# consilience-dev/llm-map-reduce-summarizer

Hardware: AMD Instinct MI355X
Metric: chunks/sec (whole node) + end-to-end wall-clock, 10h transcript, Llama-3-8B (higher is better)
Workload: dtype bf16

## Files before the change

### llm_map_reduce_summarizer_amd/csrc/kernels/stream_gemm.hip

```cpp
#include "ar_common.h"

namespace {
enum { EPI_BF16 = 0, EPI_F32_PARTIAL = 1, EPI_SWIGLU = 2, EPI_SWIGLU_SPLIT = 3, EPI_RESID_SPLIT = 4 };
constexpr int SS_PARTS = 8;
constexpr int KBLK = 128;
constexpr int LDS_XTRA = 3 * 1024;
constexpr int LDS_BUDGET = 160 * 1024 - LDS_XTRA;

struct NormArgs {
    const float* ssq;
    int ssq_tiles;
    float inv_k, eps;
    bf16* resid;
    int ldr;
    float* ssp;
    int slab_m;
    mrsum_ar::TPPush tp;
};

template <int N>
__device__ __forceinline__ void wait_vmcnt() {
    static_assert(N >= 0 && N < 64, "vmcnt range");
    __builtin_amdgcn_s_waitcnt((N & 15) | (7 << 4) | (15 << 8) | ((N >> 4) << 14));
}
// ... 560 lines not shown
        case 6: L8(MT_, EPI_, 6); break;            \
        case 7: L8(MT_, EPI_, 7); break;            \
        default: L8(MT_, EPI_, 8); break;           \
    }
#define BY_EPI8(MT_)                                                      \
    if (epi == EPI_BF16) { BY_WPB8(MT_, EPI_BF16) }                       \
    else if (epi == EPI_F32_PARTIAL) { BY_WPB8(MT_, EPI_F32_PARTIAL) }    \
    else if (epi == EPI_SWIGLU) { BY_WPB8(MT_, EPI_SWIGLU) }              \
    else if (epi == EPI_SWIGLU_SPLIT) { BY_WPB8(MT_, EPI_SWIGLU_SPLIT) }  \
    else { BY_WPB8(MT_, EPI_RESID_SPLIT) }
    switch (mt) {
        case 1: BY_EPI8(1); break;
        case 2: BY_EPI8(2); break;
        case 3: BY_EPI8(3); break;
        default: BY_EPI8(4); break;
    }
#undef BY_EPI8
#undef BY_WPB8
#undef L8
    return (int)hipGetLastError();
}

namespace {
constexpr int P14_TILE = 3584, P14_NIB = 2048, P14_TWO = 3072;
typedef unsigned int u32x2 __attribute__((ext_vector_type(2)));

template <int AUX = 0>
__device__ __forceinline__ void glds4(const void* g, char* lds) {
    __builtin_amdgcn_global_load_lds((const __attribute__((address_space(1))) void*)g,
                                     (__attribute__((address_space(3))) void*)lds, 4, 0, AUX);
}

template <int Q>
__device__ __forceinline__ uint32_t p14_hi4(uint32_t q4, uint32_t s2, uint32_t base4) {
    constexpr int SS = Q == 3 ? 7 : Q;
    const uint32_t c5 = q4 | ((s2 << Q) & 0x10101010u);
    const uint32_t nz = (c5 + 0x1f1f1f1fu) & 0x20202020u;
    const uint32_t on = (nz << 3) - (nz >> 5);
    return (c5 + (on & base4)) | ((s2 << SS) & 0x80808080u);
}

template <int PAR>
__device__ __forceinline__ bf16x8 p14_frag(uint32_t l0, uint32_t l1, uint32_t nb, uint32_t s2, uint32_t base4) {
    const uint32_t h0 = p14_hi4<2 * PAR>(nb & 0x0f0f0f0fu, s2, base4);
    const uint32_t h1 = p14_hi4<2 * PAR + 1>((nb >> 4) & 0x0f0f0f0fu, s2, base4);
    const u32x4 o = {__builtin_amdgcn_perm(h0, l0, 0x05010400u), __builtin_amdgcn_perm(h0, l0, 0x07030602u),
                     __builtin_amdgcn_perm(h1, l1, 0x05010400u), __builtin_amdgcn_perm(h1, l1, 0x07030602u)};
    return __builtin_bit_cast(bf16x8, o);
}
}

template <int MT, int EPI, int WPB>
__global__ __launch_bounds__(64 * WPB, 1) void stream_p14_kernel(const bf16* __restrict__ x, int ldx,
                                                                 const unsigned char* __restrict__ W, int base7,
                                                                 int K, int M, void* __restrict__ out, int ldo,
                                                                 int kper, float* __restrict__ parts,
                                                                 int* __restrict__ counters, const NormArgs e) {
    constexpr int R = 16 * WPB, BM = 16 * MT;
    constexpr int WBYTES = WPB * P14_TILE, SLOT = WBYTES + BM * 256;
    constexpr int D = (LDS_BUDGET / SLOT) < 8 ? (LDS_BUDGET / SLOT) : 8;
    static_assert(D >= 2, "ring too shallow");
    constexpr int XP = 2 * BM / 8;
    constexpr int XI = (XP + WPB - 1) / WPB;
    constexpr int NI = 5 + XI;
    static_assert(NI * (D - 2) < 64, "vmcnt range");
    __shared__ __attribute__((aligned(1024))) char lds[D * SLOT + LDS_XTRA];
    float* const s_ss = reinterpret_cast<float*>(lds + D * SLOT + 1024);

    const int tid = threadIdx.x, lane = tid & 63, w = tid >> 6;
    const int n0 = blockIdx.x * R;
    const int ks = blockIdx.y * kper;
    const int nkb = kper / KBLK;

    const unsigned char* const wsrc = W + ((size_t)(n0 / 16 + w) * (K / KBLK) + ks / KBLK) * P14_TILE;
    const int prow = lane >> 3, pslot = lane & 7;
    const bf16* xsrc[XI];
    int xdst[XI];
#pragma unroll
    for (int i = 0; i < XI; ++i) {
        const int q = w + WPB * i;
        const int qq = q < XP ? q : 0;
        const int row = 8 * (qq >> 1) + prow;
        xsrc[i] = x + (size_t)min(row, M - 1) * ldx + ks + 8 * (8 * (qq & 1) + (pslot ^ prow));
        xdst[i] = q < XP ? WBYTES + q * 1024 : -1;
    }
#define ISSUE14(slot, kb)                                                                            \
    {                                                                                                \
        char* base = lds + (slot) * SLOT;                                                            \
        char* wb = base + w * P14_TILE;                                                              \
        const unsigned char* ws = wsrc + (size_t)(kb) * P14_TILE;                                    \
        glds16<2>(ws + 16 * lane, wb);                                                               \
        glds16<2>(ws + 1024 + 16 * lane, wb + 1024);                                                 \
        glds16<2>(ws + P14_NIB + 16 * lane, wb + P14_NIB);                                           \
        glds4<2>(ws + P14_TWO + 4 * lane, wb + P14_TWO);                                             \
        glds4<2>(ws + P14_TWO + 256 + 4 * lane, wb + P14_TWO + 256);                                 \
        _Pragma("unroll") for (int i = 0; i < XI; ++i)                                               \
            glds16(xsrc[i] + (kb) * KBLK, xdst[i] >= 0 ? base + xdst[i] : lds + D * SLOT);           \
    }

    f32x4 acc[MT];
#pragma unroll
    for (int m = 0; m < MT; ++m) acc[m] = f32x4{0.f, 0.f, 0.f, 0.f};

#pragma unroll
    for (int s = 0; s < D - 1; ++s) ISSUE14(s, min(s, nkb - 1));

    const uint32_t base4 = (uint32_t)(base7 - 1) * 0x01010101u;
    const int r = lane & 15, g = lane >> 4;
    for (int j = 0; j < nkb; ++j) {
        if (j + D - 2 < nkb) wait_vmcnt<NI * (D - 2)>();
        else wait_vmcnt<0>();
        raw_barrier();
        if (j + D - 1 < nkb) ISSUE14((j + D - 1) % D, j + D - 1);
        const char* wl = lds + (j % D) * SLOT + w * P14_TILE;
        const char* xl = lds + (j % D) * SLOT + WBYTES;
        const u32x4 lo0 = *reinterpret_cast<const u32x4*>(wl + 16 * lane);
        const u32x4 lo1 = *reinterpret_cast<const u32x4*>(wl + 1024 + 16 * lane);
        const u32x4 nb = *reinterpret_cast<const u32x4*>(wl + P14_NIB + 16 * lane);
        const u32x2 s2 = *reinterpret_cast<const u32x2*>(wl + P14_TWO + 8 * lane);
        bf16x8 av[4];
        av[0] = p14_frag<0>(lo0[0], lo0[1], nb[0], s2.x, base4);
        av[1] = p14_frag<1>(lo0[2], lo0[3], nb[1], s2.x, base4);
        av[2] = p14_frag<0>(lo1[0], lo1[1], nb[2], s2.y, base4);
        av[3] = p14_frag<1>(lo1[2], lo1[3], nb[3], s2.y, base4);
#pragma unroll
        for (int i = 0; i < 4; ++i) {
#pragma unroll
            for (int m = 0; m < MT; ++m) {
                const u32x4 bv = *reinterpret_cast<const u32x4*>(xl + img_off(16 * m + r, 4 * i + g));
                acc[m] = __builtin_amdgcn_mfma_f32_16x16x32_bf16(av[i], __builtin_bit_cast(bf16x8, bv), acc[m], 0, 0, 0);
            }
        }
    }
#undef ISSUE14

    stream_epilogue<MT, EPI, WPB>(acc, lds, s_ss, n0, M, out, ldo, parts, counters, e);
}

MRSUM_API int mrsum_stream_p14(const void* x, int ldx, const void* W, int base7, int N, int K, int M, void* out,
                               int ldo, int epi, int splits, int wpb, void* parts, int* counters, const float* ssq,
                               int ssq_tiles, float eps, void* resid, int ldr, float* ssp, void* ar, hipStream_t s) {
    if (M <= 0) return 0;
    if (wpb < 4 || wpb > 8 || M > 64 || K % KBLK || N % (16 * wpb) || splits < 1 || (K / KBLK) % splits ||
        epi < EPI_BF16 || epi > EPI_RESID_SPLIT || base7 < 1 || base7 > 97 || ar)
        return (int)hipErrorInvalidValue;
    const bool split_epi = epi == EPI_SWIGLU_SPLIT || epi == EPI_RESID_SPLIT;
    if (epi != EPI_F32_PARTIAL && !split_epi && splits != 1) return (int)hipErrorInvalidValue;
    if (split_epi && (!parts || !counters)) return (int)hipErrorInvalidValue;
    if (epi == EPI_RESID_SPLIT && (!resid || !ssp || ldr % 4)) return (int)hipErrorInvalidValue;
    if (ssq && (ssq_tiles <= 0 || ssq_tiles % (4 * SS_PARTS))) return (int)hipErrorInvalidValue;
    NormArgs e;
    e.ssq = ssq; e.ssq_tiles = ssq_tiles; e.inv_k = 1.f / (float)K; e.eps = eps;
    e.resid = (bf16*)resid; e.ldr = ldr; e.ssp = ssp; e.slab_m = 0;
    e.tp = mrsum_ar::tp_push_of(nullptr);
    const int kper = K / splits;
    const int mt = (M + 15) / 16;
    dim3 grid(N / (16 * wpb), splits), block(64 * wpb);
    auto X = (const bf16*)x;
    auto Wp = (const unsigned char*)W;
    auto P = (float*)parts;
#define L14(MT_, EPI_, WPB_) \
    stream_p14_kernel<MT_, EPI_, WPB_><<<grid, block, 0, s>>>(X, ldx, Wp, base7, K, M, out, ldo, kper, P, counters, e)
#define BY_WPB14(MT_, EPI_)                         \
    switch (wpb) {                                  \
        case 4: L14(MT_, EPI_, 4); break;           \
        case 5: L14(MT_, EPI_, 5); break;           \
        case 6: L14(MT_, EPI_, 6); break;           \
        case 7: L14(MT_, EPI_, 7); break;           \
        default: L14(MT_, EPI_, 8); break;          \
    }
#define BY_EPI14(MT_)                                                      \
    if (epi == EPI_BF16) { BY_WPB14(MT_, EPI_BF16) }                       \
    else if (epi == EPI_F32_PARTIAL) { BY_WPB14(MT_, EPI_F32_PARTIAL) }    \
    else if (epi == EPI_SWIGLU) { BY_WPB14(MT_, EPI_SWIGLU) }              \
    else if (epi == EPI_SWIGLU_SPLIT) { BY_WPB14(MT_, EPI_SWIGLU_SPLIT) }  \
    else { BY_WPB14(MT_, EPI_RESID_SPLIT) }
    switch (mt) {
        case 1: BY_EPI14(1); break;
        case 2: BY_EPI14(2); break;
        case 3: BY_EPI14(3); break;
        default: BY_EPI14(4); break;
    }
#undef BY_EPI14
#undef BY_WPB14
#undef L14
    return (int)hipGetLastError();
}

namespace {
__global__ __launch_bounds__(256) void p14_max_kernel(const uint4* __restrict__ W, size_t n16, int* __restrict__ stats) {
    uint32_t m = 0;
    for (size_t i = (size_t)blockIdx.x * blockDim.x + threadIdx.x; i < n16; i += (size_t)gridDim.x * blockDim.x) {
        const uint4 v = W[i];
        const uint32_t d[4] = {v.x, v.y, v.z, v.w};
#pragma unroll
        for (int c = 0; c < 4; ++c) m = max(m, max((d[c] >> 8) & 0x7fu, (d[c] >> 24) & 0x7fu));
    }
#pragma unroll
    for (int o = 32; o > 0; o >>= 1) m = max(m, (uint32_t)__shfl_xor((int)m, o, 64));
    if ((threadIdx.x & 63) == 0) atomicMax(stats, (int)m);
}

__global__ __launch_bounds__(64) void p14_pack_kernel(const bf16* __restrict__ W, int K, unsigned char* __restrict__ P,
                                                      int* __restrict__ stats) {
    const int lane = threadIdx.x, r = lane & 15, g = lane >> 4;
    const int nkb = K / KBLK;
    const size_t tile = blockIdx.x;
    const int G = (int)(tile / nkb), kb = (int)(tile % nkb);
    const int base7 = max(stats[0] - 30, 1);
    const uint4* src = reinterpret_cast<const uint4*>(W + (size_t)(16 * G + r) * K + (size_t)kb * KBLK + 8 * g);
    uint32_t lo[8], nb[4], s2[2] = {0u, 0u};
// ... 15 lines not shown
            s2[i >> 1] |= (c5 >> 4) << (8 * b + 4 - q) | sg << (8 * b + 7 - (q == 3 ? 7 : q));
        }
    }
    unsigned char* t = P + tile * P14_TILE;
    *reinterpret_cast<uint4*>(t + 16 * lane) = make_uint4(lo[0], lo[1], lo[2], lo[3]);
    *reinterpret_cast<uint4*>(t + 1024 + 16 * lane) = make_uint4(lo[4], lo[5], lo[6], lo[7]);
    *reinterpret_cast<uint4*>(t + P14_NIB + 16 * lane) = make_uint4(nb[0], nb[1], nb[2], nb[3]);
    *reinterpret_cast<uint2*>(t + P14_TWO + 8 * lane) = make_uint2(s2[0], s2[1]);
    if (bad) atomicAdd(stats + 1, bad);
}
}

MRSUM_API int mrsum_p14_pack(const void* W, int N, int K, void* packed, int* stats, hipStream_t s) {
    if (N <= 0 || K <= 0 || N % 16 || K % KBLK || !W || !packed || !stats) return (int)hipErrorInvalidValue;
    hipError_t rc = hipMemsetAsync(stats, 0, 2 * sizeof(int), s);
    if (rc != hipSuccess) return (int)rc;
    const size_t n16 = (size_t)N * K / 8;
    const int blocks = (int)((n16 + 255) / 256 < 4096 ? (n16 + 255) / 256 : 4096);
    p14_max_kernel<<<blocks, 256, 0, s>>>((const uint4*)W, n16, stats);
    p14_pack_kernel<<<(unsigned)((size_t)(N / 16) * (K / KBLK)), 64, 0, s>>>((const bf16*)W, K, (unsigned char*)packed,
                                                                              stats);
    return (int)hipGetLastError();
}
```

### llm_map_reduce_summarizer_amd/engine/model.py

```python

from __future__ import annotations

import hashlib
import math
import os
from dataclasses import dataclass
from typing import Callable, List, Optional

import torch

from .. import ops
from ..ops.reference import Fp8Weight, interleave_gate_up, rope_cos_sin
from ..parallel.dist import AsyncWorks
from .config import ModelConfig


def _seed_for(seed: int, name: str) -> int:
    return int.from_bytes(hashlib.sha1(("%d:%s" % (seed, name)).encode()).digest()[:8], "little") & ((1 << 63) - 1)


def _randn(shape, std: float, seed: int, name: str, device, dtype) -> torch.Tensor:
    g = torch.Generator(device=device)
    g.manual_seed(_seed_for(seed, name))
    t = torch.randn(*shape, generator=g, device=device, dtype=torch.float32 if device.type == "cpu" else dtype)
    t.mul_(std)
    return t.to(dtype)


# ... 142 lines not shown
            self.layers.append(LayerWeights(ones(), wqkv, wo, ones(), wgu, wd))
        self.final_norm = ones()
        lm = _randn((c.vocab_size, c.hidden), std, seed, "lm_head", dev, dt)
        v = self.vocab_local
        self.lm_head = lm[r * v:(r + 1) * v].contiguous()
        del lm
        self._quantize_lm_head()

    def _quantize_lm_head(self) -> None:
        if self.weight_dtype == "fp8" and not isinstance(self.lm_head, Fp8Weight):
            self.lm_head = Fp8Weight.quantize(self.lm_head)

    def _pack_p14(self) -> None:
        self.p14 = []
        if self.weight_dtype != "bf16" or self.tp_size != 1 or self.device.type != "cuda" \
                or self.dtype != torch.bfloat16:
            return
        hip = _hip()
        if not hip.p14_enabled():
            return
        todo = [(self.lm_head, "lm_head")]
        for lw in self.layers:
            todo += [(lw.wqkv, "qkv"), (lw.wo, "o"), (lw.wgu, "gate_up"), (lw.wdown, "down")]
        for w, role in todo:
            if hip.p14_role_used(role) and w.shape[0] % 16 == 0 and w.shape[1] % 128 == 0:
                self.p14.append(hip.p14_attach(w, role))

    def __del__(self):
        try:
            for pw in getattr(self, "p14", ()):
                _hip().p14_detach(pw.w)
        except Exception:
            pass

    def weight_bytes(self) -> int:
        def nb(t):
            return t.nbytes() if isinstance(t, Fp8Weight) else t.numel() * t.element_size()
        n = nb(self.embed) + nb(self.lm_head) + nb(self.final_norm) + sum(pw.nbytes() for pw in self.p14)
        for lw in self.layers:
            n += sum(nb(t) for t in (lw.ln1, lw.wqkv, lw.wo, lw.ln2, lw.wgu, lw.wdown))
        return n

    def local_push(self):
        if self._local_push is None:
            from ..parallel.custom_ar import LocalPush
            self._local_push = LocalPush()
        return self._local_push

    def _all_reduce(self, t: torch.Tensor) -> torch.Tensor:
        if self.tp_size > 1:
            if self.custom_ar is not None and self.custom_ar.fits(t):
                self.custom_ar.all_reduce(t)
            else:
                if t.is_cuda and torch.cuda.is_current_stream_capturing():
# ... 228 lines not shown
```

### llm_map_reduce_summarizer_amd/ops/hip.py

```python

from __future__ import annotations

import ctypes
import os
from typing import Optional

import torch

from ._lib import kernels_lib
from .reference import Fp8Weight

_c_int, _c_float, _vp = ctypes.c_int, ctypes.c_float, ctypes.c_void_p

_SIGS = {
    "mrsum_rmsnorm": [_vp, _vp, _vp, _c_int, _c_int, _c_int, _c_int, _c_float, _vp],
    "mrsum_add_rmsnorm": [_vp, _vp, _vp, _vp, _c_int, _c_int, _c_int, _c_int, _c_float, _vp],
    "mrsum_rmsnorm_fp8": [_vp, _vp, _vp, _vp, _vp, _c_int, _c_int, _c_int, _c_int, _c_float, _c_int, _vp],
    "mrsum_rope_kv": [_vp, _c_int, _c_int, _vp, _vp, _vp, _c_int, _vp, _vp, _vp, _c_int, _c_int, _c_int, _c_int,
                      _c_int, _c_int, _vp],
    "mrsum_rope_kv_parts": [_vp, _c_int, _vp, _c_int, _c_int, _vp, _vp, _vp, _c_int, _vp, _vp, _vp, _c_int,
                            _c_int, _c_int, _c_int, _c_int, _vp],
    "mrsum_swiglu": [_vp, _vp, _c_int, _c_int, _vp],
    "mrsum_kv_scatter": [_vp, _c_int, _c_int, _c_int, _vp, _vp, _vp, _vp, _c_int, _vp],
    "mrsum_embed": [_vp, _vp, _vp, _c_int, _c_int, _c_int, _vp],
    "mrsum_attn_prefill": [_vp, _c_int, _vp, _vp, _c_int, _c_int, _vp, _c_int, _c_int, _c_int, _c_int, _c_float, _vp],
    "mrsum_attn_prefill_paged": [_vp, _c_int, _vp, _vp, _c_int, _c_int, _vp, _c_int, _c_int, _c_int, _c_int, _c_float,
                                 _vp,
                                 _vp, _vp, _c_int, _vp, _vp, _c_int, _vp],
    "mrsum_attn_decode_mfma": [_vp, _c_int, _vp, _vp, _vp, _c_int, _vp, _vp, _vp, _vp, _c_int, _c_int, _c_int,
                               _c_int, _c_int, _c_int, _c_int, _c_float, _vp, _c_int, _vp],
    "mrsum_attn_decode_rope": [_vp, _c_int, _vp, _vp, _vp, _vp, _c_int, _vp, _vp, _vp, _vp, _c_int, _c_int,
                               _c_int, _c_int, _c_int, _c_int, _c_int, _c_float, _vp, _c_int, _vp],
    "mrsum_skinny_gemm": [_vp, _c_int, _vp, _c_int, _c_int, _c_int, _vp, _c_int, _c_int, _c_int, _c_int, _vp, _c_int,
                          _c_float, _vp, _c_int, _vp, _vp, _c_int, _vp],
    "mrsum_skinny_resid_capacity_w": [_c_int],
    "mrsum_skinny_lds": [_vp, _c_int, _vp, _c_int, _c_int, _c_int, _vp, _c_int, _c_int, _c_int, _c_int, _vp],
    "mrsum_stream_gemm": [_vp, _c_int, _vp, _c_int, _c_int, _c_int, _vp, _c_int, _c_int, _c_int, _c_int, _vp, _vp,
                          _vp, _c_int, _c_float, _vp, _c_int, _vp, _c_int, _vp, _vp],
    "mrsum_stream_fp8": [_vp, _c_int, _vp, _vp, _c_int, _c_int, _c_int, _vp, _c_int, _c_int, _c_int, _c_int, _vp, _vp,
                         _vp, _c_int, _c_float, _vp, _c_int, _vp, _vp, _vp],
    "mrsum_stream_p14": [_vp, _c_int, _vp, _c_int, _c_int, _c_int, _c_int, _vp, _c_int, _c_int, _c_int, _c_int, _vp,
                         _vp, _vp, _c_int, _c_float, _vp, _c_int, _vp, _vp, _vp],
    "mrsum_p14_pack": [_vp, _c_int, _c_int, _vp, _vp, _vp],
    "mrsum_skinny_fp8": [_vp, _c_int, _vp, _vp, _c_int, _c_int, _c_int, _vp, _c_int, _c_int, _c_int, _c_int, _vp,
                         _c_int, _c_float, _vp, _c_int, _vp, _vp, _c_int, _vp],
    "mrsum_skinny_fp8_resid_capacity": [],
    "mrsum_quant_fp8_rows": [_vp, _c_int, _vp, _vp, _c_int, _c_int, _vp],
    "mrsum_add_rmsnorm_parts": [_vp, _c_int, _vp, _vp, _vp, _c_int, _c_int, _c_int, _c_float, _vp],
    "mrsum_sample_keys": [_vp, _c_int, _c_int, _c_int, _c_int, _vp, _vp, _vp, _vp, _vp],
    "mrsum_sample_finish": [_vp, _vp, _vp, _vp, _vp, _vp, _c_int, _vp, _vp, _c_int, _vp],
    "mrsum_gemm": [_vp, _c_int, _vp, _c_int, _vp, _c_int, _c_int, _c_int, _c_int, _c_int, _c_int, _vp, _vp, _c_int,
                   _c_int, _vp],
    "mrsum_sample": [_vp, _c_int, _c_int, _c_int, _vp, _vp, _vp, _vp, _vp, _vp, _vp, _vp, _vp, _c_int, _vp, _vp,
                     _vp],
    "mrsum_penalize": [_vp, _c_int, _c_int, _c_int, _c_int, _vp, _c_int, _vp, _vp, _vp, _vp, _vp, _vp],
    "mrsum_penalize_scan": [_vp, _c_int, _c_int, _c_int, _c_int, _vp, _c_int, _vp, _vp, _vp, _vp, _vp, _vp],
    "mrsum_constrain": [_vp, _c_int, _c_int, _c_int, _c_int, _vp, _vp, _c_int, _vp, _vp, _vp, _vp, _vp, _vp, _vp],
    "mrsum_sample_finish_stops": [_vp, _vp, _vp, _vp, _vp, _vp, _c_int, _vp, _vp, _vp, _c_int, _vp],
    "mrsum_sample_keys_filtered": [_vp, _c_int, _c_int, _c_int, _vp, _vp, _vp, _vp, _vp, _vp, _vp, _vp, _vp, _vp],
    "mrsum_logprobs": [_vp, _c_int, _c_int, _c_int, _vp, _vp, _vp, _c_int, _vp, _vp, _vp, _vp, _vp, _vp, _vp, _vp],
    "mrsum_logprobs_pick": [_vp, _c_int, _c_int, _c_int, _vp, _c_int, _vp, _vp, _vp, _vp, _c_int, _vp],
    "mrsum_sample_thresh": [_vp, _c_int, _c_int, _c_int, _vp, _vp, _vp, _vp, _vp, _vp, _vp],
    "mrsum_sample_filtered": [_vp, _c_int, _c_int, _c_int, _vp, _vp, _vp, _vp, _vp, _vp, _vp, _vp, _vp, _vp, _vp,
                              _vp, _vp, _c_int, _vp, _vp, _vp],
}

# ... 825 lines not shown
            continue
        grid = N // (16 * wpb) * splits
        k = (round(grid / (-(-grid // N_CU) * N_CU), 3), wpb)
        if key is None or k > key:
            best, key = wpb, k
    return best


def _stream_launch(x, w, out, epi, splits, ldo, wpb, parts, counters, norm, resid, ssp, slab_m, ar=None):
    M, K = x.shape
    N = w.shape[0]
    _req(w.is_contiguous() and w.shape[1] == K, "stream_gemm: weight must be [N, K] contiguous")
    tall_ok = M <= 128 and epi in (EPI_BF16, EPI_F32_PARTIAL, EPI_SWIGLU) and norm is None
    _req(1 <= M and (M <= SKINNY_MAX_M or tall_ok) and K % 128 == 0 and 4 <= wpb <= 8 and N % (16 * wpb) == 0
         and (K // 128) % splits == 0, "stream_gemm: unsupported shape M=%d N=%d K=%d S=%d wpb=%d"
         % (M, N, K, splits, wpb))
    if epi in (EPI_SWIGLU_SPLIT, EPI_RESID_SPLIT):
        _req(parts is not None and parts.shape == (splits, M, N) and parts.dtype == torch.float32
             and counters is not None and counters.numel() >= N // (16 * wpb), "stream_gemm: split-K scratch")
    if epi == EPI_RESID_SPLIT:
        _req(ssp.shape[1] == N // (16 * wpb), "stream_gemm: ssp tiles")
    sq, tiles, eps = _norm_args(x, norm)
    rp, ldr, sp = _resid_args(x, N, epi, resid, ssp)
    pw = p14_lookup(w) if _P14 else None
    if pw is not None and M <= SKINNY_MAX_M and not slab_m and ar is None and p14_takes(pw.role, M):
        STATS["stream_p14"] += 1
        _check(_fn("mrsum_stream_p14")(_p(x), x.stride(0), _p(pw.packed), pw.base7, N, K, M, _p(out), ldo, epi, splits,
                                       wpb, _p(parts), _p(counters), sq, tiles, eps, rp, ldr, sp, None, _stream()),
               "stream_p14")
        return out
    STATS["stream_bf16"] += 1
    _check(_fn("mrsum_stream_gemm")(_p(x), x.stride(0), _p(w), N, K, M, _p(out), ldo, epi, splits, wpb, _p(parts),
                                    _p(counters), sq, tiles, eps, rp, ldr, sp, slab_m, ar, _stream()), "stream_gemm")
    return out


P14_ROLES = ("qkv", "o", "gate_up", "down", "lm_head")
_P14_PLAN = {("gate_up", 1), ("gate_up", 16), ("gate_up", 64), ("lm_head", 1), ("lm_head", 16),
             ("down", 1), ("down", 16)}
_P14 = {}


class PackedWeight:

    def __init__(self, w: torch.Tensor, packed: Optional[torch.Tensor], base7: int, packable: bool, role: str):
        self.w, self.packed, self.base7, self.packable, self.role = w, packed, base7, packable, role

    def nbytes(self) -> int:
# ... 28 lines not shown
    stats = torch.zeros(2, dtype=torch.int32, device=w.device)
    _check(_fn("mrsum_p14_pack")(_p(w), N, K, _p(packed), _p(stats), _stream()), "p14_pack")
    mx, bad = (int(v) for v in stats.tolist())
    return packed, max(mx - 30, 1), bad


def p14_attach(w: torch.Tensor, role: str) -> PackedWeight:
    _req(role in P14_ROLES, "p14_attach: unknown role %r" % (role,))
    packed, base7, bad = p14_pack(w)
    if bad:
        print("p14: %s weight %s has %d elements outside the exponent window: bf16 kernel kept"
              % (role, tuple(w.shape), bad))
        return PackedWeight(w, None, base7, False, role)
    pw = _P14[(w.data_ptr(), w.shape[0], w.shape[1])] = PackedWeight(w, packed, base7, True, role)
    return pw


def p14_detach(w: torch.Tensor) -> None:
    _P14.pop((w.data_ptr(), w.shape[0], w.shape[1]), None)


def p14_lookup(w: torch.Tensor) -> Optional[PackedWeight]:
    return _P14.get((w.data_ptr(), w.shape[0], w.shape[1]))


def linear_takes_norm(M: int, N: int, K: int) -> bool:
    return 1 <= M <= SKINNY_MAX_M and K % 128 == 0 and stream_config(N, K, splits=1) is not None


def linear(x: torch.Tensor, w: torch.Tensor, out: Optional[torch.Tensor] = None, norm=None) -> torch.Tensor:
    M, K = x.shape
    N = w.shape[0]
    _req(norm is None or linear_takes_norm(M, N, K), "linear: a deferred norm needs a stream-GEMM shape")
    tall = (SKINNY_MAX_M < M <= STREAM_TALL_M and K % 128 == 0 and norm is None
            and stream_config(N, K, splits=1) is not None and tall_wpb(N, M, 1) is not None)
    if (M > SKINNY_MAX_M and not tall) or M == 0 or K % 128:
        return gemm(x, w, out=out)
    if out is None:
        out = torch.empty(M, N, dtype=x.dtype, device=x.device)
    _req(out.is_contiguous() and out.shape == (M, N), "linear: bad out")
    if tall:
        return _stream_gemm(x, w, out, EPI_BF16, 1, N, tall_wpb(N, M, 1))
    cfg = stream_config(N, K, splits=1)
    if cfg is not None:
        return _stream_gemm(x, w, out, EPI_BF16, 1, N, cfg[0], norm=norm)
    nt = 2 if N % 32 == 0 and N >= 16384 else 1
# ... 113 lines not shown
        return _skinny_lds(x, w_gu, out, EPI_SWIGLU, 1, F2 // 2)
    return _skinny(x, w_gu, out, EPI_SWIGLU, 1, 1, F2 // 2, norm=norm)


def add_rmsnorm_parts(parts: torch.Tensor, residual: torch.Tensor, w: torch.Tensor, eps: float,
                      out: Optional[torch.Tensor] = None) -> torch.Tensor:
    _req(parts.is_cuda and parts.dtype == torch.float32 and parts.is_contiguous() and parts.dim() == 3,
         "add_rmsnorm_parts: parts must be fp32 [S, T, D]")
    _bf16_cuda(residual, w)
    S, T, D = parts.shape
    _req(residual.shape == (T, D) and residual.is_contiguous() and w.numel() == D and w.is_contiguous()
         and D % 8 == 0 and D <= 16384, "add_rmsnorm_parts: shapes")
    if out is None:
        out = torch.empty(T, D, dtype=residual.dtype, device=residual.device)
    _bf16_cuda(out)
    _rows_ok(out)
    _req(out.shape == (T, D), "add_rmsnorm_parts: bad out shape")
    _check(_fn("mrsum_add_rmsnorm_parts")(_p(parts), S, _p(residual), _p(w), _p(out), T, D, out.stride(0), eps,
                                          _stream()), "add_rmsnorm_parts")
    return out


N_CU = 256
STATS = {"tp_push": 0, "stream_p14": 0, "stream_bf16": 0}


def stream_config(N: int, K: int, swiglu: bool = False, splits: Optional[int] = None, max_splits: int = 16):
    if K % 128:
        return None
    nkb = K // 128
    best, best_key = None, None
    for wpb in (4, 5, 6, 7, 8):
        if N % (16 * wpb):
            continue
        tiles = N // (16 * wpb)
        cands = [1] if swiglu else ([splits] if splits else range(1, max_splits + 1))
        for S in cands:
            if nkb % S:
                continue
            grid = tiles * S
            eff = grid / (-(-grid // N_CU) * N_CU)
            key = (round(eff, 3), -S, wpb if grid <= 2 * N_CU else -wpb)
            if best_key is None or key > best_key:
                best, best_key = (wpb, S), key
    if best is None or best_key[0] < 0.7:
        return None
    return best
# ... 247 lines not shown
```

### llm_map_reduce_summarizer_amd/ops/reference.py

```python

from __future__ import annotations

import math
from typing import Optional

import torch

LOG2E = 1.4426950408889634


def rmsnorm(x: torch.Tensor, w: torch.Tensor, eps: float, out: Optional[torch.Tensor] = None) -> torch.Tensor:
    xf = x.float()
    y = xf * torch.rsqrt(xf.pow(2).mean(-1, keepdim=True) + eps) * w.float()
    y = y.to(x.dtype)
    if out is not None:
        out.copy_(y)
        return out
    return y


def add_rmsnorm(x: torch.Tensor, residual: torch.Tensor, w: torch.Tensor, eps: float,
                out: Optional[torch.Tensor] = None) -> torch.Tensor:
    residual.copy_((x.float() + residual.float()).to(residual.dtype))
    return rmsnorm(residual, w, eps, out)
# ... 199 lines not shown
            b, q = e & 3, 2 * (i & 1) + (e >> 2)
            two[:, :, i >> 1] |= (c5[:, :, i, e] >> 4) << (8 * b + 4 - q)
            two[:, :, i >> 1] |= sg[:, :, i, e] << (8 * b + 7 - _P14_SIGN_SHIFT[q])
    two = torch.stack([(two >> (8 * k)) & 0xff for k in range(4)], dim=-1).reshape(T, 512)
    return torch.cat([lo, nib, two], dim=1).to(torch.uint8).reshape(-1), base7, bad


def p14_unpack_ref(packed: torch.Tensor, base7: int, N: int, K: int) -> torch.Tensor:
    t = packed.reshape(-1, P14_TILE).to(torch.int64)
    T = t.shape[0]
    lo = t[:, :2048].reshape(T, 2, 64, 2, 8).permute(0, 2, 1, 3, 4).reshape(T, 64, 4, 8)
    nb = t[:, 2048:3072].reshape(T, 64, 4, 4)
    q4 = torch.cat([nb & 15, nb >> 4], dim=-1)
    tb = t[:, 3072:].reshape(T, 64, 2, 4)
    two = sum(tb[..., k] << (8 * k) for k in range(4))
    hi = torch.zeros_like(lo)
    for i in range(4):
        for e in range(8):
            b, q = e & 3, 2 * (i & 1) + (e >> 2)
            s = two[:, :, i >> 1]
            c5 = q4[:, :, i, e] | ((s >> (8 * b + 4 - q)) & 1) << 4
            e7 = torch.where(c5 == 0, c5, c5 + base7 - 1)
            hi[:, :, i, e] = ((s >> (8 * b + 7 - _P14_SIGN_SHIFT[q])) & 1) << 7 | e7
    u = (hi << 8 | lo).reshape(N // 16, K // 128, 4, 16, 4, 8).permute(0, 3, 1, 4, 2, 5).reshape(N, K)
    u = torch.where(u >= 0x8000, u - 0x10000, u)
    return u.to(torch.int16).view(torch.bfloat16)


def linear(x: torch.Tensor, w) -> torch.Tensor:
    if isinstance(w, Fp8Weight):
        return (x.float() @ w.dequant().t()).to(x.dtype)
    return torch.nn.functional.linear(x, w)


def linear_parts(x: torch.Tensor, w: torch.Tensor, splits: int = 1) -> torch.Tensor:
    K = x.shape[1]
    ks = K // splits
    wf = w.dequant() if isinstance(w, Fp8Weight) else w.float()
    return torch.stack([x[:, i * ks:(i + 1) * ks].float() @ wf[:, i * ks:(i + 1) * ks].t()
                        for i in range(splits)])


def linear_swiglu(x: torch.Tensor, w_gu) -> torch.Tensor:
    return swiglu(linear(x, w_gu))


# ... 271 lines not shown
```

Measured before the change: 2.246.

## Add lossless 13-bit packed weight format with sparse exponent exceptions for skinny GEMMs

Introduces a 13-bit packed bf16 weight layout: low mantissa byte, a 4-bit exponent code relative to a per-matrix base, and a sign bit. Rare exponents below the window are stored in a small per-row-group exception list and patched into fragments in registers. This cuts weight bytes streamed per tile from 3584 to 3328 for the memory-bound decode GEMMs (gate_up, down, lm_head), at the cost of extra ALU work and a per-iteration exception check. Matrices with more than 8 exceptions in any row group fall back to the 14-bit path, and the new path is enabled by default.

```diff
diff --git a/llm_map_reduce_summarizer_amd/csrc/kernels/stream_gemm.hip b/llm_map_reduce_summarizer_amd/csrc/kernels/stream_gemm.hip
--- a/llm_map_reduce_summarizer_amd/csrc/kernels/stream_gemm.hip
+++ b/llm_map_reduce_summarizer_amd/csrc/kernels/stream_gemm.hip
@@ -606,7 +606,12 @@
 }
 
 namespace {
-constexpr int P14_TILE = 3584, P14_NIB = 2048, P14_TWO = 3072;
+constexpr int P13_EXCAP = 8;
+template <int BITS> struct Packed;
+template <> struct Packed<14> { enum { TILE = 3584, NIB = 2048, TOP = 3072, NW = 5, WINDOW = 31 }; };
+template <> struct Packed<13> { enum { TILE = 3328, NIB = 2048, TOP = 3072, NW = 4, WINDOW = 15 }; };
+constexpr int P14_TILE = Packed<14>::TILE, P14_NIB = Packed<14>::NIB, P14_TWO = Packed<14>::TOP;
+constexpr int P13_TILE = Packed<13>::TILE, P13_NIB = Packed<13>::NIB, P13_SGN = Packed<13>::TOP;
 typedef unsigned int u32x2 __attribute__((ext_vector_type(2)));
 
 template <int AUX = 0>
@@ -624,29 +629,50 @@
     return (c5 + (on & base4)) | ((s2 << SS) & 0x80808080u);
 }
 
+__device__ __forceinline__ u32x4 packed_weave(uint32_t h0, uint32_t h1, uint32_t l0, uint32_t l1) {
+    return u32x4{__builtin_amdgcn_perm(h0, l0, 0x05010400u), __builtin_amdgcn_perm(h0, l0, 0x07030602u),
+                 __builtin_amdgcn_perm(h1, l1, 0x05010400u), __builtin_amdgcn_perm(h1, l1, 0x07030602u)};
+}
+
 template <int PAR>
-__device__ __forceinline__ bf16x8 p14_frag(uint32_t l0, uint32_t l1, uint32_t nb, uint32_t s2, uint32_t base4) {
+__device__ __forceinline__ u32x4 p14_frag(uint32_t l0, uint32_t l1, uint32_t nb, uint32_t s2, uint32_t base4) {
     const uint32_t h0 = p14_hi4<2 * PAR>(nb & 0x0f0f0f0fu, s2, base4);
     const uint32_t h1 = p14_hi4<2 * PAR + 1>((nb >> 4) & 0x0f0f0f0fu, s2, base4);
-    const u32x4 o = {__builtin_amdgcn_perm(h0, l0, 0x05010400u), __builtin_amdgcn_perm(h0, l0, 0x07030602u),
-                     __builtin_amdgcn_perm(h1, l1, 0x05010400u), __builtin_amdgcn_perm(h1, l1, 0x07030602u)};
-    return __builtin_bit_cast(bf16x8, o);
-}
-}
-
-template <int MT, int EPI, int WPB>
-__global__ __launch_bounds__(64 * WPB, 1) void stream_p14_kernel(const bf16* __restrict__ x, int ldx,
-                                                                 const unsigned char* __restrict__ W, int base7,
-                                                                 int K, int M, void* __restrict__ out, int ldo,
-                                                                 int kper, float* __restrict__ parts,
-                                                                 int* __restrict__ counters, const NormArgs e) {
+    return packed_weave(h0, h1, l0, l1);
+}
+
+template <int Q>
+__device__ __forceinline__ uint32_t p13_hi4(uint32_t q4, uint32_t sg, uint32_t base4) {
+    const uint32_t nz = (q4 + 0x0f0f0f0fu) & 0x10101010u;
+    const uint32_t on = (nz << 4) - (nz >> 4);
+    return (q4 + (on & base4)) | ((sg << (7 - Q)) & 0x80808080u);
+}
+
+template <int I>
+__device__ __forceinline__ u32x4 p13_frag(uint32_t l0, uint32_t l1, uint32_t nb, uint32_t sg, uint32_t base4) {
+    const uint32_t h0 = p13_hi4<2 * I>(nb & 0x0f0f0f0fu, sg, base4);
+    const uint32_t h1 = p13_hi4<2 * I + 1>((nb >> 4) & 0x0f0f0f0fu, sg, base4);
+    return packed_weave(h0, h1, l0, l1);
+}
+}
+
+template <int BITS, int MT, int EPI, int WPB>
+__global__ __launch_bounds__(64 * WPB, 1) void stream_packed_kernel(const bf16* __restrict__ x, int ldx,
+                                                                    const unsigned char* __restrict__ W, int base7,
+                                                                    const int* __restrict__ exoff,
+                                                                    const uint32_t* __restrict__ exlist,
+                                                                    int K, int M, void* __restrict__ out, int ldo,
+                                                                    int kper, float* __restrict__ parts,
+                                                                    int* __restrict__ counters, const NormArgs e) {
+    using F = Packed<BITS>;
+    constexpr int TILE = F::TILE;
     constexpr int R = 16 * WPB, BM = 16 * MT;
-    constexpr int WBYTES = WPB * P14_TILE, SLOT = WBYTES + BM * 256;
+    constexpr int WBYTES = WPB * TILE, SLOT = WBYTES + BM * 256;
     constexpr int D = (LDS_BUDGET / SLOT) < 8 ? (LDS_BUDGET / SLOT) : 8;
     static_assert(D >= 2, "ring too shallow");
     constexpr int XP = 2 * BM / 8;
     constexpr int XI = (XP + WPB - 1) / WPB;
-    constexpr int NI = 5 + XI;
+    constexpr int NI = F::NW + XI;
     static_assert(NI * (D - 2) < 64, "vmcnt range");
     __shared__ __attribute__((aligned(1024))) char lds[D * SLOT + LDS_XTRA];
     float* const s_ss = reinterpret_cast<float*>(lds + D * SLOT + 1024);
@@ -656,7 +682,14 @@
     const int ks = blockIdx.y * kper;
     const int nkb = kper / KBLK;
 
-    const unsigned char* const wsrc = W + ((size_t)(n0 / 16 + w) * (K / KBLK) + ks / KBLK) * P14_TILE;
+    int ex0 = 0, nex = 0;
+    if constexpr (BITS == 13) {
+        const int G = n0 / 16 + __builtin_amdgcn_readfirstlane(w);
+        ex0 = exoff[G];
+        nex = exoff[G + 1] - ex0;
+    }
+
+    const unsigned char* const wsrc = W + ((size_t)(n0 / 16 + w) * (K / KBLK) + ks / KBLK) * TILE;
     const int prow = lane >> 3, pslot = lane & 7;
     const bf16* xsrc[XI];
     int xdst[XI];
@@ -668,16 +701,16 @@
         xsrc[i] = x + (size_t)min(row, M - 1) * ldx + ks + 8 * (8 * (qq & 1) + (pslot ^ prow));
         xdst[i] = q < XP ? WBYTES + q * 1024 : -1;
     }
-#define ISSUE14(slot, kb)                                                                            \
+#define ISSUEP(slot, kb)                                                                             \
     {                                                                                                \
         char* base = lds + (slot) * SLOT;                                                            \
-        char* wb = base + w * P14_TILE;                                                              \
-        const unsigned char* ws = wsrc + (size_t)(kb) * P14_TILE;                                    \
+        char* wb = base + w * TILE;                                                                  \
+        const unsigned char* ws = wsrc + (size_t)(kb) * TILE;                                        \
         glds16<2>(ws + 16 * lane, wb);                                                               \
         glds16<2>(ws + 1024 + 16 * lane, wb + 1024);                                                 \
-        glds16<2>(ws + P14_NIB + 16 * lane, wb + P14_NIB);                                           \
-        glds4<2>(ws + P14_TWO + 4 * lane, wb + P14_TWO);                                             \
-        glds4<2>(ws + P14_TWO + 256 + 4 * lane, wb + P14_TWO + 256);                                 \
+        glds16<2>(ws + F::NIB + 16 * lane, wb + F::NIB);                                             \
+        glds4<2>(ws + F::TOP + 4 * lane, wb + F::TOP);                                               \
+        if constexpr (BITS == 14) glds4<2>(ws + F::TOP + 256 + 4 * lane, wb + F::TOP + 256);         \
         _Pragma("unroll") for (int i = 0; i < XI; ++i)                                               \
             glds16(xsrc[i] + (kb) * KBLK, xdst[i] >= 0 ? base + xdst[i] : lds + D * SLOT);           \
     }
@@ -687,7 +720,22 @@
     for (int m = 0; m < MT; ++m) acc[m] = f32x4{0.f, 0.f, 0.f, 0.f};
 
 #pragma unroll
-    for (int s = 0; s < D - 1; ++s) ISSUE14(s, min(s, nkb - 1));
+    for (int s = 0; s < D - 1; ++s) ISSUEP(s, min(s, nkb - 1));
+
+    const uint32_t kb0 = (uint32_t)(ks / KBLK);
+    uint32_t ex[P13_EXCAP], exkb = ~0u;
+    if constexpr (BITS == 13) {
+#pragma unroll
+        for (int c = 0; c < P13_EXCAP; ++c) ex[c] = ~0u;
+        if (nex > 0) {
+#pragma unroll
+            for (int c = 0; c < P13_EXCAP; ++c) {
+                if (c < nex) ex[c] = __builtin_amdgcn_readfirstlane(exlist[ex0 + c]);
+                const uint32_t kbc = ex[c] >> 18;
+                if (kbc >= kb0) exkb = min(exkb, kbc);
+            }
+        }
+    }
 
     const uint32_t base4 = (uint32_t)(base7 - 1) * 0x01010101u;
     const int r = lane & 15, g = lane >> 4;
@@ -695,39 +743,71 @@
         if (j + D - 2 < nkb) wait_vmcnt<NI * (D - 2)>();
         else wait_vmcnt<0>();
         raw_barrier();
-        if (j + D - 1 < nkb) ISSUE14((j + D - 1) % D, j + D - 1);
-        const char* wl = lds + (j % D) * SLOT + w * P14_TILE;
+        if (j + D - 1 < nkb) ISSUEP((j + D - 1) % D, j + D - 1);
+        const char* wl = lds + (j % D) * SLOT + w * TILE;
         const char* xl = lds + (j % D) * SLOT + WBYTES;
         const u32x4 lo0 = *reinterpret_cast<const u32x4*>(wl + 16 * lane);
         const u32x4 lo1 = *reinterpret_cast<const u32x4*>(wl + 1024 + 16 * lane);
-        const u32x4 nb = *reinterpret_cast<const u32x4*>(wl + P14_NIB + 16 * lane);
-        const u32x2 s2 = *reinterpret_cast<const u32x2*>(wl + P14_TWO + 8 * lane);
-        bf16x8 av[4];
-        av[0] = p14_frag<0>(lo0[0], lo0[1], nb[0], s2.x, base4);
-        av[1] = p14_frag<1>(lo0[2], lo0[3], nb[1], s2.x, base4);
-        av[2] = p14_frag<0>(lo1[0], lo1[1], nb[2], s2.y, base4);
-        av[3] = p14_frag<1>(lo1[2], lo1[3], nb[3], s2.y, base4);
+        const u32x4 nb = *reinterpret_cast<const u32x4*>(wl + F::NIB + 16 * lane);
+        u32x4 av[4];
+        if constexpr (BITS == 14) {
+            const u32x2 s2 = *reinterpret_cast<const u32x2*>(wl + F::TOP + 8 * lane);
+            av[0] = p14_frag<0>(lo0[0], lo0[1], nb[0], s2.x, base4);
+            av[1] = p14_frag<1>(lo0[2], lo0[3], nb[1], s2.x, base4);
+            av[2] = p14_frag<0>(lo1[0], lo1[1], nb[2], s2.y, base4);
+            av[3] = p14_frag<1>(lo1[2], lo1[3], nb[3], s2.y, base4);
+        } else {
+            const uint32_t sg = *reinterpret_cast<const uint32_t*>(wl + F::TOP + 4 * lane);
+            av[0] = p13_frag<0>(lo0[0], lo0[1], nb[0], sg, base4);
+            av[1] = p13_frag<1>(lo0[2], lo0[3], nb[1], sg, base4);
+            av[2] = p13_frag<2>(lo1[0], lo1[1], nb[2], sg, base4);
+            av[3] = p13_frag<3>(lo1[2], lo1[3], nb[3], sg, base4);
+            if (kb0 + (uint32_t)j == exkb) {
+                const uint32_t cur = exkb;
+                exkb = ~0u;
+#pragma unroll
+                for (int c = 0; c < P13_EXCAP; ++c) {
+                    uint32_t xc = ex[c];
+                    asm volatile("" : "+s"(xc));
+                    const uint32_t kbc = xc >> 18;
+                    if (kbc == cur) {
+                        const int sl = (xc >> 7) & 31;
+                        const uint32_t v = lane == (int)((xc >> 12) & 63) ? (xc & 127u) << (8 + 16 * (sl & 1)) : 0u;
+#pragma unroll
+                        for (int i = 0; i < 4; ++i)
+#pragma unroll
+                            for (int d = 0; d < 4; ++d) av[i][d] |= sl >> 1 == 4 * i + d ? v : 0u;
+                    } else if (kbc > cur) {
+                        exkb = min(exkb, kbc);
+                    }
+                }
+            }
+        }
 #pragma unroll
         for (int i = 0; i < 4; ++i) {
 #pragma unroll
             for (int m = 0; m < MT; ++m) {
                 const u32x4 bv = *reinterpret_cast<const u32x4*>(xl + img_off(16 * m + r, 4 * i + g));
-                acc[m] = __builtin_amdgcn_mfma_f32_16x16x32_bf16(av[i], __builtin_bit_cast(bf16x8, bv), acc[m], 0, 0, 0);
-            }
-        }
-    }
-#undef ISSUE14
+                acc[m] = __builtin_amdgcn_mfma_f32_16x16x32_bf16(__builtin_bit_cast(bf16x8, av[i]),
+                                                                 __builtin_bit_cast(bf16x8, bv), acc[m], 0, 0, 0);
+            }
+        }
+    }
+#undef ISSUEP
 
     stream_epilogue<MT, EPI, WPB>(acc, lds, s_ss, n0, M, out, ldo, parts, counters, e);
 }
 
-MRSUM_API int mrsum_stream_p14(const void* x, int ldx, const void* W, int base7, int N, int K, int M, void* out,
-                               int ldo, int epi, int splits, int wpb, void* parts, int* counters, const float* ssq,
-                               int ssq_tiles, float eps, void* resid, int ldr, float* ssp, void* ar, hipStream_t s) {
+template <int BITS>
+static int launch_packed(const void* x, int ldx, const void* W, int base7, const int* exoff, const uint32_t* exlist,
+                         int N, int K, int M, void* out, int ldo, int epi, int splits, int wpb, void* parts,
+                         int* counters, const float* ssq, int ssq_tiles, float eps, void* resid, int ldr, float* ssp,
+                         void* ar, hipStream_t s) {
     if (M <= 0) return 0;
     if (wpb < 4 || wpb > 8 || M > 64 || K % KBLK || N % (16 * wpb) || splits < 1 || (K / KBLK) % splits ||
-        epi < EPI_BF16 || epi > EPI_RESID_SPLIT || base7 < 1 || base7 > 97 || ar)
+        epi < EPI_BF16 || epi > EPI_RESID_SPLIT || base7 < 1 || base7 > 128 - Packed<BITS>::WINDOW || ar)
         return (int)hipErrorInvalidValue;
+    if (BITS == 13 && (!exoff || !exlist || K / KBLK >= 0x3fff)) return (int)hipErrorInvalidValue;
     const bool split_epi = epi == EPI_SWIGLU_SPLIT || epi == EPI_RESID_SPLIT;
     if (epi != EPI_F32_PARTIAL && !split_epi && splits != 1) return (int)hipErrorInvalidValue;
     if (split_epi && (!parts || !counters)) return (int)hipErrorInvalidValue;
@@ -743,8 +823,9 @@
     auto X = (const bf16*)x;
     auto Wp = (const unsigned char*)W;
     auto P = (float*)parts;
-#define L14(MT_, EPI_, WPB_) \
-    stream_p14_kernel<MT_, EPI_, WPB_><<<grid, block, 0, s>>>(X, ldx, Wp, base7, K, M, out, ldo, kper, P, counters, e)
+#define L14(MT_, EPI_, WPB_)                                                                                      \
+    stream_packed_kernel<BITS, MT_, EPI_, WPB_><<<grid, block, 0, s>>>(X, ldx, Wp, base7, exoff, exlist, K, M, out, \
+                                                                       ldo, kper, P, counters, e)
 #define BY_WPB14(MT_, EPI_)                         \
     switch (wpb) {                                  \
         case 4: L14(MT_, EPI_, 4); break;           \
@@ -771,6 +852,21 @@
     return (int)hipGetLastError();
 }
 
+MRSUM_API int mrsum_stream_p14(const void* x, int ldx, const void* W, int base7, int N, int K, int M, void* out,
+                               int ldo, int epi, int splits, int wpb, void* parts, int* counters, const float* ssq,
+                               int ssq_tiles, float eps, void* resid, int ldr, float* ssp, void* ar, hipStream_t s) {
+    return launch_packed<14>(x, ldx, W, base7, nullptr, nullptr, N, K, M, out, ldo, epi, splits, wpb, parts, counters,
+                             ssq, ssq_tiles, eps, resid, ldr, ssp, ar, s);
+}
+
+MRSUM_API int mrsum_stream_p13(const void* x, int ldx, const void* W, int base7, const int* exoff,
+                               const unsigned int* exlist, int N, int K, int M, void* out, int ldo, int epi, int splits,
+                               int wpb, void* parts, int* counters, const float* ssq, int ssq_tiles, float eps,
+                               void* resid, int ldr, float* ssp, void* ar, hipStream_t s) {
+    return launch_packed<13>(x, ldx, W, base7, exoff, exlist, N, K, M, out, ldo, epi, splits, wpb, parts, counters,
+                             ssq, ssq_tiles, eps, resid, ldr, ssp, ar, s);
+}
+
 namespace {
 __global__ __launch_bounds__(256) void p14_max_kernel(const uint4* __restrict__ W, size_t n16, int* __restrict__ stats) {
     uint32_t m = 0;
@@ -832,3 +928,63 @@
                                                                               stats);
     return (int)hipGetLastError();
 }
+
+namespace {
+__global__ __launch_bounds__(64) void p13_pack_kernel(const bf16* __restrict__ W, int K, unsigned char* __restrict__ P,
+                                                      int* __restrict__ stats, int* __restrict__ excnt,
+                                                      uint32_t* __restrict__ exbuf) {
+    const int lane = threadIdx.x, r = lane & 15, g = lane >> 4;
+    const int nkb = K / KBLK;
+    const size_t tile = blockIdx.x;
+    const int G = (int)(tile / nkb), kb = (int)(tile % nkb);
+    const int base7 = max(stats[0] - 14, 1);
+    const uint4* src = reinterpret_cast<const uint4*>(W + (size_t)(16 * G + r) * K + (size_t)kb * KBLK + 8 * g);
+    uint32_t lo[8], nb[4], sg = 0u;
+    int nexc = 0;
+#pragma unroll
+    for (int i = 0; i < 4; ++i) {
+        const uint4 v = src[4 * i];
+        const uint32_t d[4] = {v.x, v.y, v.z, v.w};
+        lo[2 * i] = lo[2 * i + 1] = nb[i] = 0u;
+#pragma unroll
+        for (int el = 0; el < 8; ++el) {
+            const uint32_t wv = (d[el >> 1] >> (16 * (el & 1))) & 0xffffu;
+            const int e7 = (wv >> 8) & 0x7f;
+            const bool exc = e7 != 0 && e7 < base7;
+            const uint32_t c4 = e7 == 0 || exc ? 0u : (uint32_t)(e7 - base7 + 1);
+            if (exc) {
+                ++nexc;
+                const int at = atomicAdd(excnt + G, 1);
+                if (at < P13_EXCAP)
+                    exbuf[(size_t)G * P13_EXCAP + at] = (uint32_t)kb << 18 | (uint32_t)lane << 12 |
+                                                        (uint32_t)(8 * i + el) << 7 | (uint32_t)e7;
+            }
+            const int b = el & 3;
+            lo[2 * i + (el >> 2)] |= (wv & 0xffu) << (8 * b);
+            nb[i] |= c4 << (8 * b + 4 * (el >> 2));
+            sg |= (wv >> 15) << (8 * b + 2 * i + (el >> 2));
+        }
+    }
+    unsigned char* t = P + tile * P13_TILE;
+    *reinterpret_cast<uint4*>(t + 16 * lane) = make_uint4(lo[0], lo[1], lo[2], lo[3]);
+    *reinterpret_cast<uint4*>(t + 1024 + 16 * lane) = make_uint4(lo[4], lo[5], lo[6], lo[7]);
+    *reinterpret_cast<uint4*>(t + P13_NIB + 16 * lane) = make_uint4(nb[0], nb[1], nb[2], nb[3]);
+    *reinterpret_cast<uint32_t*>(t + P13_SGN + 4 * lane) = sg;
+    if (nexc) atomicAdd(stats + 1, nexc);
+}
+}
+
+MRSUM_API int mrsum_p13_pack(const void* W, int N, int K, void* packed, int* stats, int* excnt, unsigned int* exbuf,
+                             hipStream_t s) {
+    if (N <= 0 || K <= 0 || N % 16 || K % KBLK || K / KBLK >= 0x3fff || !W || !packed || !stats || !excnt || !exbuf)
+        return (int)hipErrorInvalidValue;
+    hipError_t rc = hipMemsetAsync(stats, 0, 2 * sizeof(int), s);
+    if (rc == hipSuccess) rc = hipMemsetAsync(excnt, 0, (size_t)(N / 16) * sizeof(int), s);
+    if (rc != hipSuccess) return (int)rc;
+    const size_t n16 = (size_t)N * K / 8;
+    const int blocks = (int)((n16 + 255) / 256 < 4096 ? (n16 + 255) / 256 : 4096);
+    p14_max_kernel<<<blocks, 256, 0, s>>>((const uint4*)W, n16, stats);
+    p13_pack_kernel<<<(unsigned)((size_t)(N / 16) * (K / KBLK)), 64, 0, s>>>((const bf16*)W, K, (unsigned char*)packed,
+                                                                              stats, excnt, exbuf);
+    return (int)hipGetLastError();
+}
diff --git a/llm_map_reduce_summarizer_amd/engine/model.py b/llm_map_reduce_summarizer_amd/engine/model.py
--- a/llm_map_reduce_summarizer_amd/engine/model.py
+++ b/llm_map_reduce_summarizer_amd/engine/model.py
@@ -4,6 +4,7 @@
 import hashlib
 import math
 import os
+import sys
 from dataclasses import dataclass
 from typing import Callable, List, Optional
 
@@ -192,14 +193,25 @@
         todo = [(self.lm_head, "lm_head")]
         for lw in self.layers:
             todo += [(lw.wqkv, "qkv"), (lw.wo, "o"), (lw.wgu, "gate_up"), (lw.wdown, "down")]
+        n13 = n14 = n16 = nex = 0
         for w, role in todo:
-            if hip.p14_role_used(role) and w.shape[0] % 16 == 0 and w.shape[1] % 128 == 0:
-                self.p14.append(hip.p14_attach(w, role))
+            if w.shape[0] % 16 or w.shape[1] % 128:
+                continue
+            pw = hip.packed_attach(w, role)
+            if pw is None:
+                continue
+            self.p14.append(pw)
+            if isinstance(pw, hip.Packed13Weight):
+                n13, nex = n13 + 1, nex + pw.nex
+            else:
+                n14, n16 = n14 + pw.packable, n16 + (not pw.packable)
+        print("packed decode weights: %d p13 (%d exceptions), %d p14, %d left bf16" % (n13, nex, n14, n16),
+              file=sys.stderr)
 
     def __del__(self):
         try:
             for pw in getattr(self, "p14", ()):
-                _hip().p14_detach(pw.w)
+                _hip().packed_detach(pw.w)
         except Exception:
             pass
 
diff --git a/llm_map_reduce_summarizer_amd/ops/hip.py b/llm_map_reduce_summarizer_amd/ops/hip.py
--- a/llm_map_reduce_summarizer_amd/ops/hip.py
+++ b/llm_map_reduce_summarizer_amd/ops/hip.py
@@ -42,6 +42,9 @@
     "mrsum_stream_p14": [_vp, _c_int, _vp, _c_int, _c_int, _c_int, _c_int, _vp, _c_int, _c_int, _c_int, _c_int, _vp,
                          _vp, _vp, _c_int, _c_float, _vp, _c_int, _vp, _vp, _vp],
     "mrsum_p14_pack": [_vp, _c_int, _c_int, _vp, _vp, _vp],
+    "mrsum_stream_p13": [_vp, _c_int, _vp, _c_int, _vp, _vp, _c_int, _c_int, _c_int, _vp, _c_int, _c_int, _c_int,
+                         _c_int, _vp, _vp, _vp, _c_int, _c_float, _vp, _c_int, _vp, _vp, _vp],
+    "mrsum_p13_pack": [_vp, _c_int, _c_int, _vp, _vp, _vp, _vp, _vp],
     "mrsum_skinny_fp8": [_vp, _c_int, _vp, _vp, _c_int, _c_int, _c_int, _vp, _c_int, _c_int, _c_int, _c_int, _vp,
                          _c_int, _c_float, _vp, _c_int, _vp, _vp, _c_int, _vp],
     "mrsum_skinny_fp8_resid_capacity": [],
@@ -913,8 +916,17 @@
         _req(ssp.shape[1] == N // (16 * wpb), "stream_gemm: ssp tiles")
     sq, tiles, eps = _norm_args(x, norm)
     rp, ldr, sp = _resid_args(x, N, epi, resid, ssp)
+    packed_ok = M <= SKINNY_MAX_M and not slab_m and ar is None
+    p3 = p13_lookup(w) if _P13 else None
+    if p3 is not None and packed_ok and p13_takes(p3.role, M):
+        STATS["stream_p14"] += 1
+        STATS["stream_p13"] += 1
+        _check(_fn("mrsum_stream_p13")(_p(x), x.stride(0), _p(p3.packed), p3.base7, _p(p3.exoff), _p(p3.exlist), N, K,
+                                       M, _p(out), ldo, epi, splits, wpb, _p(parts), _p(counters), sq, tiles, eps, rp,
+                                       ldr, sp, None, _stream()), "stream_p13")
+        return out
     pw = p14_lookup(w) if _P14 else None
-    if pw is not None and M <= SKINNY_MAX_M and not slab_m and ar is None and p14_takes(pw.role, M):
+    if pw is not None and packed_ok and p14_takes(pw.role, M):
         STATS["stream_p14"] += 1
         _check(_fn("mrsum_stream_p14")(_p(x), x.stride(0), _p(pw.packed), pw.base7, N, K, M, _p(out), ldo, epi, splits,
                                        wpb, _p(parts), _p(counters), sq, tiles, eps, rp, ldr, sp, None, _stream()),
@@ -989,6 +1001,93 @@
 
 def p14_lookup(w: torch.Tensor) -> Optional[PackedWeight]:
     return _P14.get((w.data_ptr(), w.shape[0], w.shape[1]))
+
+
+_P13_PLAN = {("gate_up", 1), ("gate_up", 16), ("gate_up", 64), ("lm_head", 1), ("lm_head", 16),
+             ("down", 1), ("down", 16)}
+_P13 = {}
+P13_EXCAP = 8
+P13_DEFAULT = "1"
+
+
+class Packed13Weight:
+
+    def __init__(self, w, packed, base7, exoff, exlist, nex, packable, role):
+        self.w, self.packed, self.base7, self.exoff, self.exlist = w, packed, base7, exoff, exlist
+        self.nex, self.packable, self.role = nex, packable, role
+
+    def nbytes(self) -> int:
+        if self.packed is None:
+            return 0
+        return self.packed.numel() + 4 * (self.exoff.numel() + self.exlist.numel())
+
+
+def p13_enabled() -> bool:
+    return p14_enabled() and os.environ.get("MRSUM_P13", P13_DEFAULT) == "1"
+
+
+def p13_role_used(role: str) -> bool:
+    return any(r == role for r, _ in _P13_PLAN)
+
+
+def p13_takes(role: str, M: int) -> bool:
+    return p13_enabled() and (role, p14_bucket(M)) in _P13_PLAN
+
+
+def p13_pack(w: torch.Tensor):
+    _bf16_cuda(w)
+    _req(w.dim() == 2 and w.is_contiguous() and w.shape[0] % 16 == 0 and w.shape[1] % 128 == 0
+         and w.shape[1] // 128 < 0x3fff, "p13_pack: expected a contiguous bf16 [16 n, 128 k] matrix")
+    N, K = w.shape
+    G = N // 16
+    packed = torch.empty(N * K // 8 * 13, dtype=torch.uint8, device=w.device)
+    stats = torch.zeros(2, dtype=torch.int32, device=w.device)
+    excnt = torch.zeros(G, dtype=torch.int32, device=w.device)
+    exbuf = torch.full((G, P13_EXCAP), -1, dtype=torch.int32, device=w.device)
+    _check(_fn("mrsum_p13_pack")(_p(w), N, K, _p(packed), _p(stats), _p(excnt), _p(exbuf), _stream()), "p13_pack")
+    mx, nex = (int(v) for v in stats.tolist())
+    exoff = torch.zeros(G + 1, dtype=torch.int32, device=w.device)
+    exlist = torch.zeros(1, dtype=torch.int32, device=w.device)
+    worst = 0
+    if nex:
+        worst = int(excnt.max())
+        kept = excnt.clamp(max=P13_EXCAP)
+        exoff[1:] = torch.cumsum(kept, 0)
+        srt = torch.sort(exbuf.to(torch.int64) & 0xffffffff, dim=1).values
+        keep = torch.arange(P13_EXCAP, device=w.device)[None, :] < kept[:, None]
+        words = srt[keep]
+        exlist = torch.where(words >= 2 ** 31, words - 2 ** 32, words).to(torch.int32).contiguous()
+    return packed, max(mx - 14, 1), exoff, exlist, nex, worst
+
+
+def p13_attach(w: torch.Tensor, role: str) -> Packed13Weight:
+    _req(role in P14_ROLES, "p13_attach: unknown role %r" % (role,))
+    packed, base7, exoff, exlist, nex, worst = p13_pack(w)
+    if worst > P13_EXCAP:
+        return Packed13Weight(w, None, base7, None, None, nex, False, role)
+    pw = _P13[(w.data_ptr(), w.shape[0], w.shape[1])] = Packed13Weight(w, packed, base7, exoff, exlist, nex, True, role)
+    return pw
+
+
+def p13_detach(w: torch.Tensor) -> None:
+    _P13.pop((w.data_ptr(), w.shape[0], w.shape[1]), None)
+
+
+def packed_attach(w: torch.Tensor, role: str):
+    if p13_enabled() and p13_role_used(role):
+        p3 = p13_attach(w, role)
+        if p3.packable:
+            return p3
+    return p14_attach(w, role) if p14_enabled() and p14_role_used(role) else None
+
+
+def packed_detach(w: torch.Tensor) -> None:
+    p13_detach(w)
+    p14_detach(w)
+
+
+def p13_lookup(w: torch.Tensor) -> Optional[Packed13Weight]:
+    return _P13.get((w.data_ptr(), w.shape[0], w.shape[1]))
 
 
 def linear_takes_norm(M: int, N: int, K: int) -> bool:
@@ -1148,7 +1247,7 @@
 
 
 N_CU = 256
-STATS = {"tp_push": 0, "stream_p14": 0, "stream_bf16": 0}
+STATS = {"tp_push": 0, "stream_p14": 0, "stream_p13": 0, "stream_bf16": 0}
 
 
 def stream_config(N: int, K: int, swiglu: bool = False, splits: Optional[int] = None, max_splits: int = 16):
diff --git a/llm_map_reduce_summarizer_amd/ops/reference.py b/llm_map_reduce_summarizer_amd/ops/reference.py
--- a/llm_map_reduce_summarizer_amd/ops/reference.py
+++ b/llm_map_reduce_summarizer_amd/ops/reference.py
@@ -245,6 +245,71 @@
             c5 = q4[:, :, i, e] | ((s >> (8 * b + 4 - q)) & 1) << 4
             e7 = torch.where(c5 == 0, c5, c5 + base7 - 1)
             hi[:, :, i, e] = ((s >> (8 * b + 7 - _P14_SIGN_SHIFT[q])) & 1) << 7 | e7
+    u = (hi << 8 | lo).reshape(N // 16, K // 128, 4, 16, 4, 8).permute(0, 3, 1, 4, 2, 5).reshape(N, K)
+    u = torch.where(u >= 0x8000, u - 0x10000, u)
+    return u.to(torch.int16).view(torch.bfloat16)
+
+
+P13_TILE = 3328
+P13_WINDOW = 15
+P13_EXCAP = 8
+
+
+def p13_base7(w: torch.Tensor) -> int:
+    return max(int(((p14_bits(w) >> 8) & 0x7f).max()) - (P13_WINDOW - 1), 1)
+
+
+def p13_pack_ref(w: torch.Tensor):
+    N, K = w.shape
+    assert w.dtype == torch.bfloat16 and N % 16 == 0 and K % 128 == 0 and K // 128 < 0x3fff
+    u = _p14_lanes(p14_bits(w))
+    base7 = p13_base7(w)
+    e7 = (u >> 8) & 0x7f
+    exc = (e7 != 0) & (e7 < base7)
+    c4 = torch.where((e7 == 0) | exc, torch.zeros_like(e7), e7 - base7 + 1)
+    assert int(c4.max()) <= P13_WINDOW
+    sg = u >> 15
+    T = u.shape[0]
+    lo = (u & 0xff).reshape(T, 64, 2, 16).permute(0, 2, 1, 3).reshape(T, 2048)
+    nib = (c4[..., :4] | c4[..., 4:] << 4).reshape(T, 1024)
+    sgn = torch.zeros(T, 64, dtype=torch.int64, device=u.device)
+    for i in range(4):
+        for e in range(8):
+            sgn |= sg[:, :, i, e] << (8 * (e & 3) + 2 * i + (e >> 2))
+    sgn = torch.stack([(sgn >> (8 * k)) & 0xff for k in range(4)], dim=-1).reshape(T, 256)
+    tiles = torch.cat([lo, nib, sgn], dim=1).to(torch.uint8).reshape(-1)
+    nkb = K // 128
+    t, lane, i, e = torch.nonzero(exc, as_tuple=True)
+    word = (t % nkb) << 18 | lane << 12 | (8 * i + e) << 7 | e7[t, lane, i, e]
+    grp = t // nkb
+    order = torch.argsort(grp * 2 ** 32 + word)
+    grp, word = grp[order], word[order]
+    cnt = torch.bincount(grp, minlength=N // 16)
+    exoff = torch.zeros(N // 16 + 1, dtype=torch.int64)
+    exoff[1:] = torch.cumsum(cnt, 0)
+    exlist = torch.where(word >= 2 ** 31, word - 2 ** 32, word).to(torch.int32)
+    return tiles, base7, exoff.to(torch.int32), exlist, int(cnt.max()) if cnt.numel() else 0
+
+
+def p13_unpack_ref(packed: torch.Tensor, base7: int, exoff: torch.Tensor, exlist: torch.Tensor, N: int,
+                   K: int) -> torch.Tensor:
+    t = packed.reshape(-1, P13_TILE).to(torch.int64)
+    T = t.shape[0]
+    lo = t[:, :2048].reshape(T, 2, 64, 2, 8).permute(0, 2, 1, 3, 4).reshape(T, 64, 4, 8)
+    nb = t[:, 2048:3072].reshape(T, 64, 4, 4)
+    c4 = torch.cat([nb & 15, nb >> 4], dim=-1)
+    sb = t[:, 3072:].reshape(T, 64, 4)
+    sgn = sum(sb[..., k] << (8 * k) for k in range(4))
+    e7 = torch.where(c4 == 0, c4, c4 + base7 - 1)
+    nkb = K // 128
+    words = exlist.to(torch.int64) & 0xffffffff
+    for G in range(N // 16):
+        for x in words[int(exoff[G]):int(exoff[G + 1])].tolist():
+            e7[G * nkb + (x >> 18), (x >> 12) & 63, (x >> 10) & 3, (x >> 7) & 7] = x & 127
+    hi = torch.zeros_like(lo)
+    for i in range(4):
+        for e in range(8):
+            hi[:, :, i, e] = ((sgn >> (8 * (e & 3) + 2 * i + (e >> 2))) & 1) << 7 | e7[:, :, i, e]
     u = (hi << 8 | lo).reshape(N // 16, K // 128, 4, 16, 4, 8).permute(0, 3, 1, 4, 2, 5).reshape(N, K)
     u = torch.where(u >= 0x8000, u - 0x10000, u)
     return u.to(torch.int16).view(torch.bfloat16)
```

After: 2.283, median of 6. 1.6% higher.
